# adelacvg/diff-vits

Measured on AMD Instinct MI355X. Metric: mel_frames_per_sec_50step_dpmsolver, higher is better.
Workload: dtype bf16x3 (bf16 MFMA operands split hi+lo, 3 products, fp32 accumulate / fp32 activations); 1 GPU; B=8/GPU, C=80, T=1024, L=256, 50-step DPM-Solver++(2M) multistep, UNet1DConditionModel (128, 256, 384, 512), seeded random-init weights; global_batch=8, concurrent_sub_batches_per_gpu=1, rccl_world_size=1, parallelism=dp1 (batch-sharded, RCCL broadcast of conditioning + all-gather of mels)

## Files before the change

diff-vits_amd/_lib.py:

```python
import ctypes as C
import os
import subprocess

_HERE = os.path.dirname(os.path.abspath(__file__))
LIB_PATH = os.environ.get("DVITS_LIB_FILE") or os.path.join(_HERE, "libdvits_hip.so")
CSRC = os.path.join(_HERE, "csrc")

PREC_BF16X3, PREC_BF16 = 0, 1
SOLVER_DPMPP, SOLVER_UNIPC_BH1, SOLVER_UNIPC_BH2, SOLVER_UNIPC_VARY = 0, 1, 2, 3
SKIP = {"time_uniform": 0, "time_quadratic": 1, "logSNR": 2}
SCHEDULE = {"discrete": 0, "linear": 1, "cosine": 2}
METHOD = {"multistep": 0, "singlestep": 1, "singlestep_fixed": 2}


class UNetCfg(C.Structure):
    _fields_ = [("in_channels", C.c_int32), ("out_channels", C.c_int32), ("n_levels", C.c_int32),
                ("block_out_channels", C.c_int32 * 6), ("layers_per_block", C.c_int32), ("num_heads", C.c_int32),
                ("cross_attention_dim", C.c_int32), ("norm_num_groups", C.c_int32), ("add_embed_heads", C.c_int32),
                ("norm_eps", C.c_float)]


class PencCfg(C.Structure):
    _fields_ = [("in_channels", C.c_int32), ("hidden_channels", C.c_int32), ("out_channels", C.c_int32),
                ("n_layers", C.c_int32), ("num_heads", C.c_int32), ("ffn_kernel", C.c_int32)]
# ... 52 lines not shown
    "dv_sampler_plan_method": (C.c_int, [C.c_int32, C.c_int32, C.c_void_p, C.c_int32, C.c_double, C.c_double, C.c_int32, C.c_int32,
                                         C.c_int32, C.c_int32, C.c_int32, C.c_double, C.c_double, C.c_int32, C.POINTER(C.c_void_p)]),
    "dv_plan_times": (C.c_int, [C.c_void_p, C.POINTER(C.c_int32), C.c_void_p]),
    "dv_plan_destroy": (None, [C.c_void_p]),
    "dv_plan_info": (C.c_int, [C.c_void_p, C.POINTER(C.c_int32), C.c_void_p, C.c_void_p]),
    "dv_plan_coefs": (C.c_int, [C.c_void_p, C.POINTER(C.c_int32), C.c_void_p]),
    "dv_plan_events": (C.c_int, [C.c_void_p, C.POINTER(C.c_int32), C.c_void_p, C.POINTER(C.c_int32)]),
    "dv_sampler_run": (C.c_int, [C.c_void_p, C.c_void_p, C.c_void_p, C.c_void_p, C.c_void_p]),
    "dv_sampler_run_custom": (C.c_int, [C.c_void_p, MODEL_FN, C.c_void_p, C.c_void_p, C.c_int64, C.c_void_p]),
    "dv_plan_set_thresholding": (C.c_int, [C.c_void_p, C.c_double, C.c_double, C.c_void_p]),
    "dv_sampler_run_custom_rows": (C.c_int, [C.c_void_p, MODEL_FN, C.c_void_p, C.c_void_p, C.c_int32, C.c_int64, C.c_void_p]),
    "dv_op_dynamic_threshold": (C.c_int, [C.c_void_p, C.c_int32, C.c_int64, C.c_double, C.c_double, C.c_void_p, C.c_void_p]),
    "dv_plan_set_guidance": (C.c_int, [C.c_void_p, C.c_double, C.c_int32]),
    "dv_op_cfg_combine": (C.c_int, [C.c_void_p, C.c_void_p, C.c_int32, C.c_int64, C.c_double, C.c_void_p]),
    "dv_op_cfg_pair_in": (C.c_int, [C.c_void_p, C.c_void_p, C.c_int64, C.c_void_p]),
    "dv_plan_graph_nodes": (C.c_int, [C.c_void_p, C.POINTER(C.c_int64)]),
    "dv_op_conv1d": (C.c_int, [C.c_void_p, C.c_void_p, C.c_void_p, C.c_void_p] + [C.c_int32] * 8 + [C.c_void_p]),
    "dv_op_linear": (C.c_int, [C.c_void_p, C.c_void_p, C.c_void_p, C.c_void_p] + [C.c_int32] * 4 + [C.c_void_p]),
    "dv_op_linear_planes": (C.c_int, [C.c_void_p] * 6 + [C.c_int32] * 6 + [C.c_void_p]),
    "dv_op_group_stats": (C.c_int, [C.c_void_p, C.c_void_p, C.c_void_p] + [C.c_int32] * 4 + [C.c_float, C.c_void_p]),
    "dv_op_attention": (C.c_int, [C.c_void_p] * 5 + [C.c_int32] * 5 + [C.c_void_p]),
    "dv_op_attention_frag": (C.c_int, [C.c_void_p] * 5 + [C.c_int32] * 5 + [C.c_void_p]),
    "dv_op_conv3": (C.c_int, [C.c_void_p] * 6 + [C.c_int32] * 7 + [C.c_void_p]),
}

_lib = None


def build(force=False, verbose=False):
    if force and os.path.exists(LIB_PATH):
        os.remove(LIB_PATH)
    proc = subprocess.run(["make", "-C", CSRC, "-j", str(min(8, os.cpu_count() or 1))],
                          stdout=subprocess.PIPE, stderr=subprocess.STDOUT, text=True)
    if verbose or proc.returncode != 0:
        print(proc.stdout)
    if proc.returncode != 0 or not os.path.exists(LIB_PATH):
        raise RuntimeError("building libdvits_hip.so failed:\n" + proc.stdout[-4000:])
    return LIB_PATH


def lib():
    global _lib
    if _lib is None:
        if not os.path.exists(LIB_PATH):
            raise RuntimeError("libdvits_hip.so not found at %s — run `python -c 'import __graft_entry__ as g; "
                               "g.build()'` (or `make -C diff-vits_amd/csrc`) first; there is no fallback path"
# ... 31 lines not shown
```

diff-vits_amd/csrc/dv_common.h:

```cpp
#pragma once
#include <hip/hip_runtime.h>
#include <stdint.h>

typedef unsigned short bf16_t;

enum { DV_ZERO_PAGE_BYTES = 32768 };
enum { EPI_STORE = 0, EPI_RESIDUAL = 1, EPI_GEGLU = 2, EPI_STORE_NCT = 3 };
enum { UP_NONE = 0, UP_X2 = 1, UP_SIZE = 2 };

struct GemmSeg {
  const bf16_t* a0_hi; const bf16_t* a0_lo;
  const bf16_t* a1_hi; const bf16_t* a1_lo;
  int c0, c1;
  int taps;
  int pad;
  int nkt;
};

struct GnxParams {
  unsigned long long* xchg;
  unsigned* status;
  const float* gamma; const float* beta;
  const float* tscale; const float* tshift; int ld_t;
  int groups; float eps; int silu;
// ... 185 lines not shown
hipError_t launch_rel_attention(const RelAttnParams& p, hipStream_t st);

enum { POP_GEMM = 0, POP_ATTN = 1, POP_GN = 2, POP_SPLIT = 3 };
struct PersistSync {
  unsigned arrive[8][32];
  unsigned rank[8][32];
  unsigned error;
  unsigned pad_;
  unsigned long long ticks[1024];
};

hipError_t launch_gemm(const GemmParams& p, int precision, hipStream_t st);
hipError_t gemm_init();
bool gemm_conv3_shape_ok(const GemmParams& p);
int gemm_conv3_k(const GemmParams& p);
int gemm_conv3_split(const GemmParams& p, int n_cu);
size_t gemm_conv3_split_bytes(const GemmParams& p);
int gemm_conv3_row_tiles(const GemmParams& p, int bm);
hipError_t conv3_init();
void conv3_env_refresh();
hipError_t launch_conv3(const GemmParams& p, hipStream_t st);
bool gemm_conv3_up_ok(const GemmParams& p);
hipError_t launch_conv3_up(const GemmParams& p, hipStream_t st);
void gemm_env_refresh();
hipError_t attn_init();
hipError_t launch_attention(const AttnParams& p, hipStream_t st);

hipError_t launch_pack_input(const float* x, int cx, const float* cond, int cc, bf16_t* out_hi, bf16_t* out_lo, int cpad,
                             int B, int T, hipStream_t st,
                             unsigned long long* reset = nullptr, size_t reset_words = 0, int Tp = 0);
hipError_t launch_split(const float* in, bf16_t* hi, bf16_t* lo, int64_t n, hipStream_t st);
struct GnApplyParams {
  const float* a0; const float* a1; int c0, c1;
  const float* slab0; const float* slab1;
  const float* st16_0; const float* st16_1;
  const float* scale_in; const float* shift_in;
  const float* gamma; const float* beta; float eps; int groups;
  const float* tscale; const float* tshift; int ld_t;
  int silu;
  bf16_t* out_hi; bf16_t* out_lo; bf16_t* raw_hi; bf16_t* raw_lo;
  int B, T;
  int Tv;
};
hipError_t launch_gn_apply(const GnApplyParams& p, hipStream_t st);

struct PersistOp {
// ... 64 lines not shown
```

diff-vits_amd/csrc/engine.hip:

```cpp
#include "../../include/dvits_hip.h"
#include "dv_common.h"

#include <atomic>
#include <cmath>
#include <cstdarg>
#include <cstdio>
#include <cstdlib>
#include <cstring>
#include <functional>
#include <map>
#include <memory>
#include <string>
#include <type_traits>
#include <vector>

static thread_local char g_err[1024] = "";
int dv_fail(int code, const char* fmt, ...) {
  va_list ap;
  va_start(ap, fmt);
  vsnprintf(g_err, sizeof(g_err), fmt, ap);
  va_end(ap);
  return code;
}
extern "C" const char* dv_last_error(void) { return g_err; }
// ... 596 lines not shown
  }
  bool ff_split_on = [] { const char* e = getenv("DVITS_FF_SPLIT"); return !(e && e[0] == '0'); }();
  bool chain_ff_on = [] { const char* e = getenv("DVITS_CHAIN_FF"); return !(e && e[0] == '0'); }();
  bool chain_split_on = [] { const char* e = getenv("DVITS_CHAIN_SPLIT"); return !(e && e[0] == '0'); }();
  bool chain_xsplit_on = [] { const char* e = getenv("DVITS_CHAIN_XSPLIT"); return !(e && e[0] == '0'); }();
  bool qkv_split_on = [] { const char* e = getenv("DVITS_QKV_SPLIT"); return !(e && e[0] == '0'); }();
  int qkv_split_min_wg = [] { const char* e = getenv("DVITS_QKV_SPLIT_MIN_WG"); return e ? atoi(e) : 96; }();
  int qkv_split_min_c = [] { const char* e = getenv("DVITS_QKV_SPLIT_MIN_C"); return e ? atoi(e) : 256; }();
  bool qkv_xa_on = [] { const char* e = getenv("DVITS_QKV_XA"); return !(e && e[0] == '0'); }();
  int qkv_xa_min_c = [] { const char* e = getenv("DVITS_QKV_XA_MIN_C"); return e ? atoi(e) : 256; }();
  int ff_split_min_wg = [] { const char* e = getenv("DVITS_FF_SPLIT_MIN_WG"); return e ? atoi(e) : 96; }();
  bool gnx_ff_on = [] { const char* e = getenv("DVITS_GNX_FF"); return !(e && e[0] == '0'); }();
  bool cat_drop_fp32 = [] { const char* e = getenv("DVITS_GNX_CONCAT_KEEP_FP32"); return !(e && e[0] == '1'); }();

  int conv3_min_tiles = [] { const char* e = getenv("DVITS_CONV3_MIN_TILES"); return e ? atoi(e) : 64; }();
  int conv3_route(const GemmParams& g) const {
    if (arena.exact || autotune_on() || prec != DV_PREC_BF16X3) return 0;
    GemmParams t = g;
    t.B = B;
    if (gemm_conv3_up_ok(t)) {
      const int tu = gemm_conv3_row_tiles(t, 128) * (t.N / 64);
      return tu >= (conv3_min_tiles < 64 ? conv3_min_tiles : 96) ? 2 : 0;
    }
    if (!gemm_conv3_shape_ok(t)) return 0;
    return gemm_conv3_row_tiles(t, 64) * (t.N / 64) >= conv3_min_tiles ? 1 : 0;
  }
  bool conv3_takes(const GemmParams& g) const { return conv3_route(g) != 0; }
  void gemm(std::vector<OpFn>& ops, GemmParams g, const PackedW* pw, int k_real) {
    g.w_hi = pw->hi; g.w_lo = pw->lo; g.Kp = pw->Kp; g.N_pad = pw->N_pad;
    if (!g.bias) g.bias = pw->bias;
    g.B = B;
    g.zero_page = u->zero_page;
    const int p = prec;
    const int route = conv3_route(g);
    const bool c3 = route != 0 && (dry || g.Kp == gemm_conv3_k(g)) && frag(pw);
    g.c3_route = c3 ? route : 0;
    if (c3) { g.wf_hi = dry ? reinterpret_cast<const bf16_t*>(0x1000) : pw->fhi; g.wf_lo = dry ? reinterpret_cast<const bf16_t*>(0x1000) : pw->flo; }
    cur_kind = "gemm"; cur_flops = 2.0 * (double)g.M * (double)g.N * (double)k_real;
    {
      char buf[128];
      snprintf(buf, sizeof(buf), "M=%d N=%d K=%d taps=%d nseg=%d epi=%d stride=%d up=%d%s%s%s", g.M, g.N, k_real, g.seg[0].taps,
               g.nseg, g.epi, g.stride, g.up_mode, (g.stats || g.stats16) ? " +stats" : "", c3 ? " resident" : "",
               g.gnx.xchg ? " +gnx" : "");
      cur_desc = buf;
    }
    u->flops += dry ? 0.0 : cur_flops;
// ... 1765 lines not shown
    s.src = w_sc; s.C = Csc; s.taps = 1; s.c_pad = Csc; s.k_off = 3 * Cin;
    HIPCHK(launch_pack_weight(s, hi, lo, Kp, st));
  }
  HIPCHK(launch_relayout_frag(hi, fhi, Npad, Kp, st));
  HIPCHK(launch_relayout_frag(lo, flo, Npad, Kp, st));
  g.seg[0].a0_hi = xh; g.seg[0].a0_lo = xl;
  if (Csc > 0) { g.seg[1].a0_hi = sh; g.seg[1].a0_lo = sl; }
  g.w_hi = hi; g.w_lo = lo; g.wf_hi = fhi; g.wf_lo = flo; g.out = y; g.zero_page = zp;
  if (route == 1) {
    int dev = 0, n_cu = 0;
    (void)hipGetDevice(&dev); (void)hipDeviceGetAttribute(&n_cu, hipDeviceAttributeMultiprocessorCount, dev);
    if (gemm_conv3_split(g, n_cu) == 2 && ((g.M + 31) / 32) * ((g.N + 31) / 32) <= 4096) {
      g.sk_split = 2;
      g.sk_buf = sc.get<float>(gemm_conv3_split_bytes(g), st, false);
      g.sk_ticket = sc.get<unsigned>(4096 * sizeof(unsigned), st, true);
      if (!g.sk_buf || !g.sk_ticket) return dv_fail(DV_ERR_HIP, "dv_op_conv3: hipMalloc failed");
    }
  }
  hipError_t e = launch_gemm(g, DV_PREC_BF16X3, st);
  if (e != hipSuccess) return dv_fail(DV_ERR_HIP, "dv_op_conv3: launch failed: %s", hipGetErrorString(e));
  HIPCHK(hipStreamSynchronize(st));
  return DV_OK;
}
```

diff-vits_amd/csrc/kernels_conv.hip:

```cpp
#include "dv_common.h"
#include "dv_device.h"
#include "gnx_device.h"

#include <cstdlib>
#include <type_traits>

typedef __attribute__((ext_vector_type(8))) __bf16 bf16x8;
typedef __attribute__((ext_vector_type(16))) float f32x16;

#ifdef DV_GEMM_TRACE
__device__ unsigned long long g_c3_trace[1024 * 16];
__device__ int g_c3_sel = 0;
#define DV_C3TRACE(i) do { if (threadIdx.x == 0 && blockIdx.x < 1024 && (g_c3_sel == 0 || g_c3_sel == CIN)) g_c3_trace[blockIdx.x * 16 + (i)] = __builtin_amdgcn_s_memtime(); } while (0)
extern "C" int dv_debug_c3_trace_select(int cin) {
  hipError_t e = hipMemcpyToSymbol(HIP_SYMBOL(g_c3_sel), &cin, sizeof(cin));
  void* d = nullptr;
  if (e == hipSuccess) e = hipGetSymbolAddress(&d, HIP_SYMBOL(g_c3_trace));
  return (int)(e != hipSuccess ? e : hipMemset(d, 0, sizeof(g_c3_trace)));
}
extern "C" int dv_debug_c3_trace(unsigned long long* host, int n_wg) {
  return (int)hipMemcpyFromSymbol(host, HIP_SYMBOL(g_c3_trace), (size_t)n_wg * 16 * sizeof(unsigned long long));
}
#else
#define DV_C3TRACE(i) do {} while (0)
// ... 289 lines not shown
    };
    bf16x8 ah[2][2], al[2][2];
    read_a(0, ah[0], al[0]);
#pragma unroll
    for (int u = 0; u < G::U; ++u) {
      const int cur = u & 1;
      if (u + 1 < G::U) read_a(u + 1, ah[cur ^ 1], al[cur ^ 1]);
      const BFrag f = bq[u % G::DEPTH];
      acc[0] = __builtin_amdgcn_mfma_f32_32x32x16_bf16(f.h, al[cur][0], acc[0], 0, 0, 0);
      acc[1] = __builtin_amdgcn_mfma_f32_32x32x16_bf16(f.h, al[cur][1], acc[1], 0, 0, 0);
      acc[0] = __builtin_amdgcn_mfma_f32_32x32x16_bf16(f.l, ah[cur][0], acc[0], 0, 0, 0);
      acc[1] = __builtin_amdgcn_mfma_f32_32x32x16_bf16(f.l, ah[cur][1], acc[1], 0, 0, 0);
      acc[0] = __builtin_amdgcn_mfma_f32_32x32x16_bf16(f.h, ah[cur][0], acc[0], 0, 0, 0);
      acc[1] = __builtin_amdgcn_mfma_f32_32x32x16_bf16(f.h, ah[cur][1], acc[1], 0, 0, 0);
      __builtin_amdgcn_sched_barrier(0);
      if (u + G::DEPTH < G::U) bq[u % G::DEPTH] = load_unit(u + G::DEPTH);
      __builtin_amdgcn_sched_barrier(0);
    }
  };
  if (kq == 0) run(std::integral_constant<int, 0>{});
  else if (kq == 1) run(std::integral_constant<int, 1>{});
  else if (kq == 2) run(std::integral_constant<int, 2>{});
  else run(std::integral_constant<int, 3>{});
  DV_C3TRACE(3);

  conv3_finish(p, smem, s_bias, s_gnx, acc, rpre, tl, tid, lane, wave, CIN);
}

namespace {
constexpr int BMU = 128, RFU = 4;
template <int CIN>
struct ConvGeomU {
  static constexpr int NCH = CIN / 64, KPT = CIN / 16, KS = 3 * KPT, U = KS / 4;
  static constexpr int DEPTH = U < 6 ? U : 6;
  static constexpr int A_PL = NCH * CHP;
  static constexpr int RED = 2 * 4 * RFU * 4 * 64 * 16;
  static constexpr int SMEM = 2 * A_PL > RED ? 2 * A_PL : RED;
  static_assert(CIN % 64 == 0 && KS % 4 == 0 && SMEM + 4096 <= 160 * 1024, "geometry");
};
}

template <int CIN>
__global__ __launch_bounds__(NT) void k_conv3u(const GemmParams p) {
  using G = ConvGeomU<CIN>;
  extern __shared__ __attribute__((aligned(1024))) char smem[];
  __shared__ __attribute__((aligned(16))) float s_bias[BN];
// ... 443 lines not shown
    const int j = 2 * j2;
    read_a(NCH + j + 1, 1, ahb[1], alb[1]);
    mma(bq[2 * POS], ahb[0], alb[0]);
    __builtin_amdgcn_sched_barrier(0);
    if (!(DV_C3_EXP & 2)) bq[2 * POS] = load_ks(3 * KPT + 4 * (JA + min(j + 6, NC2 - 1)));
    __builtin_amdgcn_sched_barrier(0);
    read_a(NCH + j + 2, 1, ahb[0], alb[0]);
    if (j + 1 < NC2) mma(bq[2 * POS + 1], ahb[1], alb[1]);
    __builtin_amdgcn_sched_barrier(0);
    if (!(DV_C3_EXP & 2)) bq[2 * POS + 1] = load_ks(3 * KPT + 4 * (JA + min(j + 7, NC2 - 1)));
    __builtin_amdgcn_sched_barrier(0);
  };
  for (int j2 = 0; j2 < NS2; j2 += 3) {
    pair(j2, std::integral_constant<int, 0>{});
    if (j2 + 1 < NS2) pair(j2 + 1, std::integral_constant<int, 1>{});
    if (j2 + 2 < NS2) pair(j2 + 2, std::integral_constant<int, 2>{});
  }
  DV_C3TRACE(3);
  conv3_finish(p, smem, s_bias, s_gnx, acc, rpre, tl, tid, lane, wave, CIN);
}

static bool g_conv3_on = true;
static int g_conv3_stream = 512;
void conv3_env_refresh() {
  const char* e = getenv("DVITS_CONV3"); g_conv3_on = !(e && e[0] == '0');
  const char* e2 = getenv("DVITS_CONV3_STREAM"); g_conv3_stream = e2 ? atoi(e2) : 512;
}
static const bool g_conv3_env_once = [] { conv3_env_refresh(); return true; }();

bool gemm_conv3_shape_ok(const GemmParams& p) {
  if (!g_conv3_on || p.nseg < 1 || p.nseg > 2 || p.seg[0].taps != 3 || p.seg[0].pad != 1 || p.stride != 1 || p.up_mode != UP_NONE) return false;
  const int cin = p.seg[0].c0 + p.seg[0].c1;
  if (cin < 128 || cin > 1024 || cin % 128 != 0) return false;
  if (p.seg[0].c0 % 64 != 0 || p.seg[0].c1 % 64 != 0 || (p.seg[0].c1 > 0 && !p.seg[0].a1_hi)) return false;
  if (p.nseg == 2) {
    const GemmSeg& s1 = p.seg[1];
    if (s1.taps != 1 || s1.pad != 0 || s1.c0 <= 0 || s1.c0 % 64 != 0 || s1.c1 % 64 != 0 || (s1.c1 > 0 && !s1.a1_hi) || s1.c0 + s1.c1 > 2048) return false;
  }
  const int tv_out = p.Tv_out > 0 ? p.Tv_out : p.T_out, tv_in = p.Tv_in > 0 ? p.Tv_in : p.T_in;
  if (p.T_in != p.T_out || tv_in != tv_out || p.T_virt != tv_out || tv_out > p.T_out || tv_out <= p.T_out - 32) return false;
  if (p.T_out % 32 != 0 || p.N % BN != 0 || p.B <= 0 || p.M != p.B * p.T_out) return false;
  if ((p.epi != EPI_STORE && p.epi != EPI_RESIDUAL) || p.stats || p.rowstat_out || p.ln_stat || p.relu || p.rowmask) return false;
  if ((p.ldo & 7) != 0 || (p.epi == EPI_RESIDUAL && (p.ldres & 3) != 0) || p.force_tile != GT_AUTO) return false;
  return true;
}
int gemm_conv3_row_tiles(const GemmParams& p, int bm) { return p.B * ((p.T_out + bm - 1) / bm); }
int gemm_conv3_split(const GemmParams& p, int n_cu) {
  static const bool on = [] { const char* e = getenv("DVITS_CONV3_SPLIT"); return !(e && e[0] == '0'); }();
  if (!on || n_cu <= 0 || !gemm_conv3_shape_ok(p)) return 0;
  const int cin = p.seg[0].c0 + p.seg[0].c1, nch = cin >> 6, nc2 = p.nseg > 1 ? (p.seg[1].c0 + p.seg[1].c1) >> 6 : 0;
  if (cin <= 512 && cin <= g_conv3_stream && p.nseg == 1) return 0;
  if (2 * gemm_conv3_row_tiles(p, BM) * (p.N / BN) > n_cu || nch < 4 || nch + ((nc2 + 1) >> 1) < 8) return 0;
  return 2;
}
size_t gemm_conv3_split_bytes(const GemmParams& p) { return (size_t)2 * gemm_conv3_row_tiles(p, BM) * (p.N / BN) * BM * BN * sizeof(float); }
bool gemm_conv3_up_ok(const GemmParams& p) {
  if (!g_conv3_on || p.nseg != 1 || p.seg[0].taps != 3 || p.seg[0].pad != 1 || p.stride != 1 || p.up_mode != UP_X2) return false;
  const int cin = p.seg[0].c0 + p.seg[0].c1;
  if (cin != 128 && cin != 256 && cin != 384 && cin != 512) return false;
  if (p.seg[0].c0 % 64 != 0 || p.seg[0].c1 % 64 != 0 || (p.seg[0].c1 > 0 && !p.seg[0].a1_hi)) return false;
  const int tv_out = p.Tv_out > 0 ? p.Tv_out : p.T_out, tv_in = p.Tv_in > 0 ? p.Tv_in : p.T_in;
  if (tv_out != 2 * tv_in || p.T_virt != tv_out || tv_out > p.T_out || tv_out <= p.T_out - 32 || tv_in > p.T_in) return false;
  if (p.T_out % 32 != 0 || p.N % BN != 0 || p.B <= 0 || p.M != p.B * p.T_out) return false;
  if ((p.epi != EPI_STORE && p.epi != EPI_RESIDUAL) || p.stats || p.rowstat_out || p.ln_stat || p.relu || p.rowmask) return false;
  if ((p.ldo & 7) != 0 || (p.epi == EPI_RESIDUAL && (p.ldres & 3) != 0) || p.force_tile != GT_AUTO || p.sk_buf) return false;
  return true;
}
int gemm_conv3_k(const GemmParams& p) {
  return 3 * (p.seg[0].c0 + p.seg[0].c1) + (p.nseg > 1 ? p.seg[1].c0 + p.seg[1].c1 : 0);
}
static void conv3_geometry(GemmParams& p, int bm) {
  p.c3_tu = (p.T_out + bm - 1) / bm;
  p.c3_tu_magic = p.c3_tu <= 1 ? 0u : (unsigned)(((1ull << 32) + (unsigned)p.c3_tu - 1) / (unsigned)p.c3_tu);
}

template <int CIN>
static hipError_t conv3_launch(const GemmParams& p, hipStream_t st) {
  constexpr int smem = ConvGeom<CIN>::SMEM;
  hipLaunchKernelGGL((k_conv3<CIN>), dim3(gemm_conv3_row_tiles(p, BM) * (p.N / BN)), dim3(NT), smem, st, p);
  return hipGetLastError();
}
template <int CIN>
static hipError_t conv3_attr() {
  return hipFuncSetAttribute(reinterpret_cast<const void*>(k_conv3<CIN>), hipFuncAttributeMaxDynamicSharedMemorySize, ConvGeom<CIN>::SMEM);
}
template <int CIN>
static hipError_t conv3u_attr() {
  return hipFuncSetAttribute(reinterpret_cast<const void*>(k_conv3u<CIN>), hipFuncAttributeMaxDynamicSharedMemorySize, ConvGeomU<CIN>::SMEM);
}
template <int CIN>
static hipError_t conv3u_launch(const GemmParams& p, hipStream_t st) {
  constexpr int smem = ConvGeomU<CIN>::SMEM;
  hipLaunchKernelGGL((k_conv3u<CIN>), dim3(gemm_conv3_row_tiles(p, BMU) * (p.N / BN)), dim3(NT), smem, st, p);
  return hipGetLastError();
}
hipError_t launch_conv3_up(const GemmParams& pin, hipStream_t st) {
  GemmParams p = pin;
  if (!p.wf_hi || !p.wf_lo || !gemm_conv3_up_ok(p) || p.Kp != 3 * (p.seg[0].c0 + p.seg[0].c1) || p.sk_mode != 0) return hipErrorInvalidValue;
  if (p.Tv_out <= 0) p.Tv_out = p.T_out;
  if (p.Tv_in <= 0) p.Tv_in = p.T_in;
  conv3_geometry(p, BMU);
  if (p.xcd_n > 0) p.xcd_n = 0;
  switch (p.seg[0].c0 + p.seg[0].c1) {
    case 128: return conv3u_launch<128>(p, st);
    case 256: return conv3u_launch<256>(p, st);
    case 384: return conv3u_launch<384>(p, st);
    default: return conv3u_launch<512>(p, st);
  }
}
hipError_t conv3_init() {
  hipError_t e;
  if ((e = conv3u_attr<128>()) != hipSuccess) return e;
  if ((e = conv3u_attr<256>()) != hipSuccess) return e;
  if ((e = conv3u_attr<384>()) != hipSuccess) return e;
  if ((e = conv3u_attr<512>()) != hipSuccess) return e;
  if ((e = hipFuncSetAttribute(reinterpret_cast<const void*>(k_conv3s), hipFuncAttributeMaxDynamicSharedMemorySize, S_TOTAL)) != hipSuccess) return e;
  if ((e = conv3_attr<128>()) != hipSuccess) return e;
  if ((e = conv3_attr<256>()) != hipSuccess) return e;
  if ((e = conv3_attr<384>()) != hipSuccess) return e;
  return conv3_attr<512>();
}
hipError_t launch_conv3(const GemmParams& pin, hipStream_t st) {
  GemmParams p = pin;
  if (!p.wf_hi || !p.wf_lo || !gemm_conv3_shape_ok(p) || p.Kp != gemm_conv3_k(p) || (p.sk_mode != 0 && p.sk_mode != 3)) return hipErrorInvalidValue;
  if (p.Tv_out <= 0) p.Tv_out = p.T_out;
  if (p.Tv_in <= 0) p.Tv_in = p.T_in;
  conv3_geometry(p, BM);
  const int tiles = gemm_conv3_row_tiles(p, BM) * (p.N / BN);
  if (p.sk_mode == 3) {
    if (!p.sk_buf || !p.sk_ticket || p.sk_split != 2 || p.seg[0].c0 + p.seg[0].c1 < 256) return hipErrorInvalidValue;
    hipLaunchKernelGGL(k_conv3s, dim3(2 * tiles), dim3(NT_S), S_TOTAL, st, p);
    return hipGetLastError();
  }
  const int cin = p.seg[0].c0 + p.seg[0].c1;
  if (cin > 512 || cin > g_conv3_stream || p.nseg > 1) {
    hipLaunchKernelGGL(k_conv3s, dim3(tiles), dim3(NT_S), S_TOTAL, st, p);
    return hipGetLastError();
  }
  switch (cin) {
// ... 7 lines not shown
```

diff-vits_amd/csrc/kernels_gemm.hip:

```cpp
#include "dv_common.h"
#define DV_GEMM_TRACE_OWNER
#include "gemm_tile.h"

#include <cstdio>
#include <cstdlib>
#include <type_traits>

template <int BM, int BN, int BK, int WM, int WN, int NSPLIT, int KS>
__global__ __launch_bounds__(64 * WM * WN * KS) void k_gemm(const GemmParams p) {
  extern __shared__ __attribute__((aligned(1024))) char smem[];
  asm volatile("" ::"s"(p.seg[0].a0_hi), "s"(p.seg[1].a0_hi), "s"(p.seg[1].pad), "s"(p.T_in), "s"(p.w_hi), "s"(p.M), "s"(p.res),
               "s"(p.out_hi), "s"(p.zero_page), "s"(p.ln_u), "s"(p.gnx.xchg), "s"(p.gnx.y_hi), "s"(p.xcd_n), "s"(p.xcd_inv_tn));
  const int n_tiles_n = (p.N + BN - 1) / BN;
  const int nwg = gridDim.x;
  int bid = blockIdx.x;
  int tm0, tn0, ksel = 0;
  if (p.xcd_n > 0) {
    const int x = bid & 7, i = bid >> 3;
    const int ks_i = x >> p.xcd_sh_mn, r = x & ((1 << p.xcd_sh_mn) - 1), xm_i = r >> p.xcd_sh_n, xn_i = r & (p.xcd_n - 1);
    const int lm = (i * p.xcd_inv_tn) >> 16, ln = i - lm * p.xcd_tn;
    tm0 = (xm_i * p.xcd_tm + lm) * BM; tn0 = (xn_i * p.xcd_tn + ln) * BN; ksel = ks_i;
  } else {
    {
      const int q = nwg >> 3, r = nwg & 7, xcd = bid & 7;
// ... 183 lines not shown
    auto lg2 = [](int v) { int s2 = 0; while ((1 << s2) < v) ++s2; return s2; };
    p.xcd_n = best_xn; p.xcd_sh_n = lg2(best_xn); p.xcd_sh_mn = lg2(xm * best_xn);
    p.xcd_tn = tn / best_xn; p.xcd_tm = tm / xm; p.xcd_inv_tn = (65536 + p.xcd_tn - 1) / p.xcd_tn;
  }
}
static int gemm_utt_tiles_per_xcd(const GemmParams& p, int tu, int tm, int tn) {
  if (p.xcd_n > 0) return (tu < p.xcd_tm ? tu : p.xcd_tm) * p.xcd_tn;
  const int q = (tm * tn + 7) / 8;
  return tu * tn < q ? tu * tn : q;
}

bool gemm_handover_rounds() {
  static const bool on = [] { const char* e = getenv("DVITS_GNX_ROUNDS"); return !(e && e[0] == '0'); }();
  return on;
}
int gemm_gnx_plan(const GemmParams& p, int n_cu) {
  if (p.force_tile != GT_AUTO || (p.epi != EPI_STORE && p.epi != EPI_RESIDUAL) || !p.stats16 || p.rowmask || p.relu) return 0;
  const int skc = p.gnx.sk_c;
  if (p.M != p.B * p.T_out || p.gnx.groups <= 0 || p.gnx.groups > 64 || skc < 0 || (p.N + skc) % p.gnx.groups != 0) return 0;
  const int cpg = (p.N + skc) / p.gnx.groups;
  if (cpg % 16 != 0 || p.N % 16 != 0 || skc % 16 != 0) return 0;
  int bm, bn, tu;
  if (p.c3_route) {
    bm = p.c3_route == 2 ? 128 : 64; bn = 64;
    if (p.T_out % 32 != 0 || p.N % bn != 0) return 0;
    tu = (p.T_out + bm - 1) / bm;
  } else {
    gemm_pick_tile(p, bm, bn);
    if (p.T_out % bm != 0 || p.N % bn != 0) return 0;
    tu = p.T_out / bm;
  }
  if (skc > 0 && ((skc / 16 + p.N / bn - 1) / (p.N / bn)) * 16 > 128) return 0;
  if ((p.T_out / 32) * (cpg / 16) > 256) return 0;
  const int tm = p.B * tu, tn = p.N / bn, tiles = tm * tn;
  const bool pair = p.sk_buf && p.sk_split == 2 && p.sk_ticket;
  if (p.sk_buf && !pair) return 0;
  if (pair) {
    if (2 * tiles > n_cu) return 0;
  } else if (tiles > n_cu) {
    if (!gemm_handover_rounds() || n_cu < 8) return 0;
    GemmParams t = p;
    if (p.c3_route == 2) t.xcd_n = 0; else gemm_xcd_rect(t, tm, tn, 1);
    if (gemm_utt_tiles_per_xcd(t, tu, tm, tn) > n_cu / 8) return 0;
  }
  return (p.M / 32) * (p.N / 16);
}

// ... 14 lines not shown
      for (int s2 = 0; s2 < p.nseg; ++s2) k += p.seg[s2].taps * (p.seg[s2].c0 + p.seg[s2].c1);
      snprintf(g_trace_desc, sizeof(g_trace_desc), "M=%d N=%d K=%d taps=%d nseg=%d epi=%d stride=%d up=%d%s%s%s%s%s%s split=%d%s",
               p.M, p.N, k, p.seg[0].taps, p.nseg, p.epi, p.stride, p.up_mode, p.stats ? " +colstats" : "", p.stats16 ? " +stats16" : "",
               p.gnx.xchg ? " +gnx" : "", p.out_hi ? " +planes" : "", p.rowstat_out ? " +rowstat" : "", p.ln_stat ? " +ln" : "",
               p.sk_buf ? p.sk_split : 0, (p.sk_buf && p.sk_ticket && p.sk_split == 2) ? "f" : "");
    }
    ++g_trace_no;
  }
#endif
  const bool x3 = precision == 0;
  if (!p.zero_page || (x3 && !p.w_lo)) return hipErrorInvalidValue;
  if (p.Tv_out <= 0) p.Tv_out = p.T_out;
  if (p.Tv_in <= 0) p.Tv_in = p.T_in;
  if (p.Tv_out > p.T_out || p.Tv_in > p.T_in || ((p.stats16 || p.gnx.xchg) && p.Tv_out <= p.T_out - 32)) return hipErrorInvalidValue;
  if (p.T_out < 1 || (unsigned long long)(p.M > 0 ? p.M : 1) * (unsigned long long)p.T_out >= (1ull << 32)) return hipErrorInvalidValue;
  p.tout_magic = gemm_tout_magic(p.T_out);
  if (p.ln_stat && (p.ln_nblk < 1 || p.ln_nblk > 16)) return hipErrorInvalidValue;
  for (int s2 = 0; s2 < p.nseg; ++s2)
    if (2 * (size_t)p.seg[s2].c0 + 256 > DV_ZERO_PAGE_BYTES || 2 * (size_t)p.seg[s2].c1 + 256 > DV_ZERO_PAGE_BYTES) return hipErrorInvalidValue;
  p.c3_route = 0;
  if (x3 && p.wf_hi && p.wf_lo) {
    if (gemm_conv3_shape_ok(p) && p.Kp == gemm_conv3_k(p)) p.c3_route = 1;
    else if (gemm_conv3_up_ok(p) && p.Kp == 3 * (p.seg[0].c0 + p.seg[0].c1)) p.c3_route = 2;
  }
  if (p.gnx.xchg && p.sk_mode == 0) {
    static const int n_cu = [] { int d = 0, n = 0; (void)hipGetDevice(&d); (void)hipDeviceGetAttribute(&n, hipDeviceAttributeMultiprocessorCount, d); return n; }();
    if (!p.gnx.status || !p.gnx.y_hi || !p.gnx.gamma || !p.gnx.beta || gemm_gnx_plan(p, n_cu) <= 0) return hipErrorInvalidValue;
    if (p.gnx.sk_c > 0 && (!p.gnx.sk_x || !p.gnx.sk_stat16 || !p.gnx.sk_y_hi || (x3 && !p.gnx.sk_y_lo) || p.gnx.tscale)) return hipErrorInvalidValue;
  }
  if (p.sk_buf && p.sk_split == 2 && p.sk_ticket && p.sk_mode == 0) {
    p.sk_mode = 3;
    return launch_gemm(p, precision, st);
  }
  if (p.sk_buf && p.sk_split >= 2 && p.sk_mode == 0) {
    p.sk_mode = 1;
    hipError_t e = launch_gemm(p, precision, st);
    if (e != hipSuccess) return e;
    p.sk_mode = 2;
    return launch_gemm(p, precision, st);
  }
  if (!p.sk_buf || p.sk_split < 2) { p.sk_buf = nullptr; p.sk_split = 0; p.sk_mode = 0; p.sk_ticket = nullptr; }
  const bool c3 = p.c3_route == 1 && (p.sk_mode == 0 || p.sk_mode == 3);
  p.xcd_n = 0;
  if (p.force_tile == GT_AUTO) {
    int bm, bn;
    gemm_pick_tile(p, bm, bn);
    const int tm = c3 ? gemm_conv3_row_tiles(p, 64) : (p.M + bm - 1) / bm, tn = c3 ? p.N / 64 : (p.N + bn - 1) / bn;
    const int xs = (p.sk_mode == 1 || p.sk_mode == 3) ? p.sk_split : 1;
    gemm_xcd_rect(p, tm, tn, xs);
  }
  if (c3) return launch_conv3(p, st);
  if (p.c3_route == 2 && p.sk_mode == 0) return launch_conv3_up(p, st);
  const GemmTune& tune = gemm_tune();
  const int big_tiles = ((p.M + 127) / 128) * ((p.N + 127) / 128);
  bool k64 = tune.bk64 != 0;
  for (int s = 0; s < p.nseg; ++s) k64 = k64 && p.seg[s].c0 % 64 == 0 && p.seg[s].c1 % 64 == 0;
  const int ft = p.force_tile & 0xff;
  if (ft != GT_AUTO && (p.force_tile & GT_BK64) && !k64) return hipErrorInvalidValue;
  const bool big = ft != GT_AUTO ? ft == GT_T0 : big_tiles >= tune.big;
  const int bk = ft != GT_AUTO ? ((p.force_tile & GT_BK64) ? 64 : 32) : ((!big && k64) ? 64 : 32);
  for (int s = 0; s < p.nseg; ++s) {
    if (p.seg[s].c0 % 32 != 0 || p.seg[s].c1 % 32 != 0) return hipErrorInvalidValue;
    p.seg[s].nkt = p.seg[s].taps * (p.seg[s].c0 + p.seg[s].c1) / bk;
  }
  if (ft != GT_AUTO) return bk == 64 ? Tiles<64>::launch_forced(p, x3, ft, st) : Tiles<32>::launch_forced(p, x3, ft, st);
  if (big) return tune.ksplit ? Tiles<32>::T0::launch(p, x3, st) : Tiles<32>::T0S::launch(p, x3, st);
  if (bk == 64) return Tiles<64>::launch(p, x3, tune.min_wg, tune.ksplit != 0, st);
  return Tiles<32>::launch(p, x3, tune.min_wg > 0 ? tune.min_wg : 1, false, st);
}
```

include/dvits_hip.h:

```cpp
#ifndef DVITS_HIP_H
#define DVITS_HIP_H

#include <stdint.h>

#ifdef __cplusplus
extern "C" {
#endif

typedef enum {
  DV_OK = 0,
  DV_ERR_INVALID = -1,
  DV_ERR_HIP = -2,
  DV_ERR_STATE = -3,
  DV_ERR_MISSING_WEIGHT = -4
} dv_status;

typedef enum { DV_PREC_BF16X3 = 0, DV_PREC_BF16 = 1 } dv_precision;

typedef struct {
  int32_t in_channels;
  int32_t out_channels;
  int32_t n_levels;
  int32_t block_out_channels[6];
  int32_t layers_per_block;
// ... 116 lines not shown
int dv_tenc_forward(dv_tenc* t, const int64_t* ids, const int64_t* tone, const int64_t* language, const int64_t* lengths,
                    const float* g, float* x, float* m, float* logs, void* stream);
int dv_tenc_stats(dv_tenc* t, int64_t* n_launch, double* flops);
int dv_tenc_probe(dv_tenc* t, const char* name, float* host_out, int64_t capacity, int64_t* dims);


int dv_op_rel_attention(const float* q, const float* k, const float* v, const float* emb_k, const float* emb_v,
                        const int64_t* lengths, float* o, int32_t B, int32_t H, int32_t T, int32_t d, int32_t window, void* stream);

int dv_op_conv1d(const float* x, const float* w, const float* bias, float* y, int32_t B, int32_t Cin, int32_t T,
                 int32_t Cout, int32_t k, int32_t stride, int32_t up_T, int32_t precision, void* stream);
int dv_op_linear(const float* x, const float* w, const float* bias, float* y, int32_t M, int32_t K, int32_t N,
                 int32_t precision, void* stream);
int dv_op_linear_planes(const float* x, const float* w, const float* bias, float* y, uint16_t* y_hi, uint16_t* y_lo, int32_t M,
                        int32_t K, int32_t N, int32_t ldo, int32_t geglu, int32_t precision, void* stream);
int dv_op_group_stats(const float* x, float* mean, float* rstd, int32_t B, int32_t T, int32_t C, int32_t groups,
                      float eps, void* stream);
int dv_op_attention(const float* q, const float* k, const float* v, const float* bias, float* o, int32_t B,
                    int32_t H, int32_t Tq, int32_t Tk, int32_t d, void* stream);
int dv_op_attention_frag(const float* q, const float* k, const float* v, const float* bias, float* o, int32_t B,
                         int32_t H, int32_t Tq, int32_t Tk, int32_t d, void* stream);
int dv_op_conv3(const float* x, const float* w, const float* bias, const float* x_sc, const float* w_sc, float* y, int32_t B,
                int32_t Cin, int32_t T, int32_t Tp, int32_t Cout, int32_t Csc, int32_t up2, void* stream);
int dv_op_dynamic_threshold(float* x0_inout, int32_t rows, int64_t row_numel, double ratio, double max_val, float* s_out,
                            void* stream);
int dv_op_cfg_combine(const float* x0_pair, float* out, int32_t rows, int64_t row_numel, double scale, void* stream);
int dv_op_cfg_pair_in(const float* in, float* out, int64_t numel, void* stream);

#ifdef __cplusplus
}
#endif
#endif
```

Measured before the change: 68120 mel-frames/s.

## Add dedicated stride-2 conv3 kernel for UNet downsample convolutions

Adds k_conv3d, a resident-weight MFMA kernel specialised for stride-2, kernel-3 downsampling convolutions (Cin 128/256/384). It stages even and odd input rows in LDS so all three taps reuse them, and streams pre-relayouted bf16x3 weight fragments through a register queue. Previously these convs fell through to the generic k_gemm path. The engine routes them to the new kernel (c3_route=3) when enough tiles exist, and a standalone test entry point is added. It brings more template instances and tile-count thresholds that may leave some shapes underfilling the GPU.

```diff
diff --git a/diff-vits_amd/_lib.py b/diff-vits_amd/_lib.py
--- a/diff-vits_amd/_lib.py
+++ b/diff-vits_amd/_lib.py
@@ -98,6 +98,7 @@
     "dv_op_attention": (C.c_int, [C.c_void_p] * 5 + [C.c_int32] * 5 + [C.c_void_p]),
     "dv_op_attention_frag": (C.c_int, [C.c_void_p] * 5 + [C.c_int32] * 5 + [C.c_void_p]),
     "dv_op_conv3": (C.c_int, [C.c_void_p] * 6 + [C.c_int32] * 7 + [C.c_void_p]),
+    "dv_op_conv3_down": (C.c_int, [C.c_void_p] * 9 + [C.c_int32] * 7 + [C.c_void_p]),
 }
 
 _lib = None
diff --git a/diff-vits_amd/csrc/dv_common.h b/diff-vits_amd/csrc/dv_common.h
--- a/diff-vits_amd/csrc/dv_common.h
+++ b/diff-vits_amd/csrc/dv_common.h
@@ -231,6 +231,9 @@
 hipError_t launch_conv3(const GemmParams& p, hipStream_t st);
 bool gemm_conv3_up_ok(const GemmParams& p);
 hipError_t launch_conv3_up(const GemmParams& p, hipStream_t st);
+bool gemm_conv3_down_ok(const GemmParams& p);
+int gemm_conv3_down_bm(const GemmParams& p);
+hipError_t launch_conv3_down(const GemmParams& p, hipStream_t st);
 void gemm_env_refresh();
 hipError_t attn_init();
 hipError_t launch_attention(const AttnParams& p, hipStream_t st);
diff --git a/diff-vits_amd/csrc/engine.hip b/diff-vits_amd/csrc/engine.hip
--- a/diff-vits_amd/csrc/engine.hip
+++ b/diff-vits_amd/csrc/engine.hip
@@ -642,6 +642,8 @@
       const int tu = gemm_conv3_row_tiles(t, 128) * (t.N / 64);
       return tu >= (conv3_min_tiles < 64 ? conv3_min_tiles : 96) ? 2 : 0;
     }
+    if (gemm_conv3_down_ok(t))
+      return gemm_conv3_row_tiles(t, gemm_conv3_down_bm(t)) * (t.N / 64) >= conv3_min_tiles ? 3 : 0;
     if (!gemm_conv3_shape_ok(t)) return 0;
     return gemm_conv3_row_tiles(t, 64) * (t.N / 64) >= conv3_min_tiles ? 1 : 0;
   }
@@ -2453,3 +2455,66 @@
   HIPCHK(hipStreamSynchronize(st));
   return DV_OK;
 }
+
+extern "C" int dv_op_conv3_down(const float* x, const float* w, const float* bias, float* y, float* stat16, const float* gamma,
+                                const float* beta, uint16_t* yn_hi, uint16_t* yn_lo, int32_t B, int32_t C, int32_t T, int32_t Tp,
+                                int32_t Cout, int32_t groups, int32_t resident, void* stream) {
+  if (!x || !w || !y || B <= 0 || C <= 0 || T <= 0 || Tp < T || Cout <= 0 || C % 64 != 0 || Cout % 16 != 0)
+    return dv_fail(DV_ERR_INVALID, "dv_op_conv3_down: bad argument");
+  if (gamma && (!beta || !stat16 || !yn_hi || !yn_lo || groups <= 0)) return dv_fail(DV_ERR_INVALID, "dv_op_conv3_down: the in-launch GroupNorm needs beta, stat16, both planes and groups");
+  if (2 * (size_t)C + 256 > DV_ZERO_PAGE_BYTES) return dv_fail(DV_ERR_INVALID, "dv_op_conv3_down: C = %d exceeds one source tensor's width", C);
+  hipStream_t st = (hipStream_t)stream;
+  HIPCHK(gemm_init());
+  gemm_env_refresh();
+  HIPCHK(attn_init());
+  const int Kp = 3 * C, Npad = rup(Cout, 128), Tv_out = (T + 1) / 2, T_out = rup(Tv_out, 32);
+  GemmParams g{};
+  g.nseg = 1; g.B = B;
+  g.T_in = Tp; g.Tv_in = g.T_virt = T; g.T_out = T_out; g.Tv_out = Tv_out;
+  g.stride = 2; g.up_mode = UP_NONE;
+  g.M = B * T_out; g.N = Cout; g.epi = EPI_STORE; g.ldo = Cout; g.ldres = Cout; g.Kp = Kp; g.N_pad = Npad; g.bias = bias;
+  g.seg[0].c0 = C; g.seg[0].taps = 3; g.seg[0].pad = 1;
+  g.stats16 = stat16;
+  if (resident && !gemm_conv3_down_ok(g))
+    return dv_fail(DV_ERR_INVALID, "dv_op_conv3_down: B=%d C=%d T=%d Tp=%d Cout=%d is not a shape of the stride-2 convolution kernel "
+                   "(it would run on k_gemm)", B, C, T, Tp, Cout);
+  OpScratch sc;
+  const size_t xe = (size_t)B * Tp * C, we = (size_t)Npad * Kp;
+  bf16_t* xh = sc.get<bf16_t>(xe * 2, st, false); bf16_t* xl = sc.get<bf16_t>(xe * 2, st, false);
+  bf16_t* hi = sc.get<bf16_t>(we * 2, st, true); bf16_t* lo = sc.get<bf16_t>(we * 2, st, true);
+  bf16_t* fhi = sc.get<bf16_t>(we * 2, st, false); bf16_t* flo = sc.get<bf16_t>(we * 2, st, false);
+  bf16_t* zp = sc.get<bf16_t>(DV_ZERO_PAGE_BYTES, st, true);
+  if (!xh || !xl || !hi || !lo || !fhi || !flo || !zp) return dv_fail(DV_ERR_HIP, "dv_op_conv3_down: hipMalloc failed");
+  HIPCHK(launch_split(x, xh, xl, (int64_t)xe, st));
+  PackSpec s{};
+  s.src = w; s.N = Cout; s.kind = 1; s.C = C; s.taps = 3; s.c_pad = C; s.k_off = 0; s.n_off = 0;
+  HIPCHK(launch_pack_weight(s, hi, lo, Kp, st));
+  HIPCHK(launch_relayout_frag(hi, fhi, Npad, Kp, st));
+  HIPCHK(launch_relayout_frag(lo, flo, Npad, Kp, st));
+  g.seg[0].a0_hi = xh; g.seg[0].a0_lo = xl;
+  g.w_hi = hi; g.w_lo = lo; g.out = y; g.zero_page = zp;
+  if (resident) { g.wf_hi = fhi; g.wf_lo = flo; g.c3_route = 3; }
+  unsigned* status = nullptr;
+  if (gamma) {
+    int dev = 0, n_cu = 0;
+    (void)hipGetDevice(&dev); (void)hipDeviceGetAttribute(&n_cu, hipDeviceAttributeMultiprocessorCount, dev);
+    g.gnx.groups = groups;
+    const int nw = gemm_gnx_plan(g, n_cu);
+    if (nw <= 0) return dv_fail(DV_ERR_INVALID, "dv_op_conv3_down: the in-launch GroupNorm cannot be planned for this shape");
+    g.gnx.xchg = sc.get<unsigned long long>((size_t)nw * 8, st, false);
+    status = sc.get<unsigned>(64, st, true);
+    if (!g.gnx.xchg || !status) return dv_fail(DV_ERR_HIP, "dv_op_conv3_down: hipMalloc failed");
+    HIPCHK(hipMemsetAsync(g.gnx.xchg, 0xff, (size_t)nw * 8, st));
+    g.gnx.status = status; g.gnx.gamma = gamma; g.gnx.beta = beta; g.gnx.eps = 1e-5f; g.gnx.silu = 0; g.gnx.spin_max = 1 << 18;
+    g.gnx.y_hi = yn_hi; g.gnx.y_lo = yn_lo;
+  }
+  hipError_t e = launch_gemm(g, DV_PREC_BF16X3, st);
+  if (e != hipSuccess) return dv_fail(DV_ERR_HIP, "dv_op_conv3_down: launch failed: %s", hipGetErrorString(e));
+  HIPCHK(hipStreamSynchronize(st));
+  if (status) {
+    unsigned flag = 0;
+    HIPCHK(hipMemcpy(&flag, status, sizeof(flag), hipMemcpyDeviceToHost));
+    if (flag) return dv_fail(DV_ERR_HIP, "dv_op_conv3_down: the in-launch GroupNorm hand-over timed out");
+  }
+  return DV_OK;
+}
diff --git a/diff-vits_amd/csrc/kernels_conv.hip b/diff-vits_amd/csrc/kernels_conv.hip
--- a/diff-vits_amd/csrc/kernels_conv.hip
+++ b/diff-vits_amd/csrc/kernels_conv.hip
@@ -335,6 +335,153 @@
   else if (kq == 1) run(std::integral_constant<int, 1>{});
   else if (kq == 2) run(std::integral_constant<int, 2>{});
   else run(std::integral_constant<int, 3>{});
+  DV_C3TRACE(3);
+
+  conv3_finish(p, smem, s_bias, s_gnx, acc, rpre, tl, tid, lane, wave, CIN);
+}
+
+namespace {
+template <int CIN, int BMD>
+struct ConvGeomD {
+  static constexpr int NCH = CIN / 64, KPT = CIN / 16, KS = 3 * KPT, U = KS / 4;
+  static constexpr int RF = BMD / 32;
+  static constexpr int DEPTH = U < 8 ? U : 8;
+  static constexpr int NG = BMD / 4 + 1;
+  static constexpr int ROWS_D = 8 * NG;
+  static constexpr int CHP_D = ROWS_D * 128;
+  static constexpr int A_PL = NCH * CHP_D;
+  static constexpr int SMEM = 2 * A_PL > RED_BYTES ? 2 * A_PL : RED_BYTES;
+  static_assert(CIN % 64 == 0 && KS % 4 == 0 && (BMD == 32 || BMD == 64) && SMEM + 4096 <= 160 * 1024, "geometry");
+};
+}
+
+template <int CIN, int BMD>
+__global__ __launch_bounds__(NT) void k_conv3d(const GemmParams p) {
+  using G = ConvGeomD<CIN, BMD>;
+  extern __shared__ __attribute__((aligned(1024))) char smem[];
+  __shared__ __attribute__((aligned(16))) float s_bias[BN];
+  __shared__ GnxShared<BN> s_gnx;
+  asm volatile("" ::"s"(p.seg[0].a0_hi), "s"(p.seg[1].a0_hi), "s"(p.seg[1].pad), "s"(p.T_in), "s"(p.w_hi), "s"(p.M), "s"(p.res),
+               "s"(p.out_hi), "s"(p.zero_page), "s"(p.ln_u), "s"(p.gnx.xchg), "s"(p.gnx.y_hi), "s"(p.xcd_n), "s"(p.xcd_inv_tn), "s"(p.wf_lo));
+  DV_C3TRACE(0);
+  C3Tile tl;
+  conv3_tile(p, tl, BMD);
+  const int m0 = tl.m0, n0 = tl.n0, t0 = tl.t0;
+  const int tid = threadIdx.x, lane = tid & 63, wave = __builtin_amdgcn_readfirstlane(tid >> 6);
+  const int l31 = lane & 31, lh = lane >> 5;
+  const int cf = wave & 1, kq = wave >> 1;
+  const int e_wn = cf, e_wm = (wave >> 1) & 1, e_half = wave >> 2;
+  const unsigned a_base = (unsigned)(size_t)smem;
+  const GemmSeg& sg = p.seg[0];
+  const int c0 = sg.c0;
+  const int m_last = p.M - 1;
+
+  float rpre[8];
+  if (p.epi == EPI_RESIDUAL) {
+    const float* rp = p.res + (size_t)min(m0 + e_wm * 32 + l31, m_last) * p.ldres + n0 + e_wn * 32 + e_half * 16 + 4 * lh;
+#pragma unroll
+    for (int g = 0; g < 2; ++g) {
+      const float4 a = *reinterpret_cast<const float4*>(rp + 8 * g);
+      rpre[4 * g] = a.x; rpre[4 * g + 1] = a.y; rpre[4 * g + 2] = a.z; rpre[4 * g + 3] = a.w;
+    }
+  }
+  if (wave == 0) glds4(p.bias ? (const void*)(p.bias + n0 + lane) : (const void*)p.zero_page, (unsigned)(size_t)s_bias);
+  {
+    const int lr = lane >> 3, slot = lane & 7;
+    const size_t ms0 = (size_t)tl.bq * p.T_in;
+#pragma unroll
+    for (int gi = 0; gi < (G::NG + NWV - 1) / NWV; ++gi) {
+      const int g = wave + gi * NWV;
+      if (g < G::NG) {
+        const int r = g * 8 + lr;
+        const int f = r < BMD ? 2 * t0 + 2 * r : 2 * t0 + 2 * (r - BMD) - 1;
+        const bool ok = r <= 2 * BMD && f >= 0 && f < p.Tv_in;
+        const int sc8 = (slot ^ swz(r)) << 3;
+        const size_t e = ok ? (ms0 + (size_t)f) * c0 + sc8 : 0;
+#pragma unroll
+        for (int c = 0; c < G::NCH; ++c) {
+          const unsigned dst = a_base + (unsigned)(c * G::CHP_D + g * 1024);
+          glds16(ok ? (const void*)(sg.a0_hi + e + c * 64) : (const void*)p.zero_page, dst);
+          glds16(ok ? (const void*)(sg.a0_lo + e + c * 64) : (const void*)p.zero_page, dst + G::A_PL);
+        }
+      }
+    }
+  }
+  const size_t w_e0 = ((size_t)((n0 >> 5) + cf) * G::KS + (size_t)kq * G::U) * 512 + (size_t)lane * 8;
+  const bf16_t* const wh = p.wf_hi + w_e0;
+  const bf16_t* const wl = p.wf_lo + w_e0;
+  auto load_unit = [&](int j) {
+    BFrag f;
+    f.h = *reinterpret_cast<const bf16x8*>(wh + (size_t)j * 512);
+    f.l = *reinterpret_cast<const bf16x8*>(wl + (size_t)j * 512);
+    return f;
+  };
+  BFrag bq[G::DEPTH];
+#pragma unroll
+  for (int j = 0; j < G::DEPTH; ++j) bq[j] = load_unit(j);
+  __builtin_amdgcn_sched_barrier(0);
+  DV_C3TRACE(1);
+  wait_vmcnt<2 * G::DEPTH>();
+  __syncthreads();
+  DV_C3TRACE(2);
+
+  int rowb[G::RF][3], swl[G::RF][3];
+#pragma unroll
+  for (int rf = 0; rf < G::RF; ++rf)
+#pragma unroll
+    for (int tap = 0; tap < 3; ++tap) {
+      const int j = rf * 32 + l31, row = tap == 1 ? j : BMD + j + (tap >> 1);
+      rowb[rf][tap] = row * 128;
+      swl[rf][tap] = swz(row) ^ lh;
+    }
+  f32x16 acc[2];
+#pragma unroll
+  for (int rf = 0; rf < 2; ++rf)
+#pragma unroll
+    for (int r = 0; r < 16; ++r) acc[rf][r] = 0.f;
+  auto run = [&](auto kq_tag) __attribute__((always_inline)) {
+    constexpr int KQ = decltype(kq_tag)::value;
+    auto read_a = [&](int u, bf16x8 (&h)[G::RF], bf16x8 (&l)[G::RF]) {
+      const int ks = KQ * G::U + u, tap = ks / G::KPT, cs = ks - tap * G::KPT;
+#pragma unroll
+      for (int rf = 0; rf < G::RF; ++rf) {
+        const int off = (cs >> 2) * G::CHP_D + rowb[rf][tap] + ((((cs & 3) << 1) ^ swl[rf][tap]) << 4);
+        h[rf] = *reinterpret_cast<const bf16x8*>(smem + off);
+        l[rf] = *reinterpret_cast<const bf16x8*>(smem + G::A_PL + off);
+      }
+    };
+    bf16x8 ah[2][G::RF], al[2][G::RF];
+    read_a(0, ah[0], al[0]);
+#pragma unroll
+    for (int u = 0; u < G::U; ++u) {
+      const int cur = u & 1;
+      if (u + 1 < G::U) read_a(u + 1, ah[cur ^ 1], al[cur ^ 1]);
+      const BFrag f = bq[u % G::DEPTH];
+      if constexpr (G::RF == 2) {
+        acc[0] = __builtin_amdgcn_mfma_f32_32x32x16_bf16(f.h, al[cur][0], acc[0], 0, 0, 0);
+        acc[1] = __builtin_amdgcn_mfma_f32_32x32x16_bf16(f.h, al[cur][1], acc[1], 0, 0, 0);
+        acc[0] = __builtin_amdgcn_mfma_f32_32x32x16_bf16(f.l, ah[cur][0], acc[0], 0, 0, 0);
+        acc[1] = __builtin_amdgcn_mfma_f32_32x32x16_bf16(f.l, ah[cur][1], acc[1], 0, 0, 0);
+        acc[0] = __builtin_amdgcn_mfma_f32_32x32x16_bf16(f.h, ah[cur][0], acc[0], 0, 0, 0);
+        acc[1] = __builtin_amdgcn_mfma_f32_32x32x16_bf16(f.h, ah[cur][1], acc[1], 0, 0, 0);
+      } else {
+        acc[1] = __builtin_amdgcn_mfma_f32_32x32x16_bf16(f.h, al[cur][0], acc[1], 0, 0, 0);
+        acc[0] = __builtin_amdgcn_mfma_f32_32x32x16_bf16(f.h, ah[cur][0], acc[0], 0, 0, 0);
+        acc[1] = __builtin_amdgcn_mfma_f32_32x32x16_bf16(f.l, ah[cur][0], acc[1], 0, 0, 0);
+      }
+      __builtin_amdgcn_sched_barrier(0);
+      if (u + G::DEPTH < G::U) bq[u % G::DEPTH] = load_unit(u + G::DEPTH);
+      __builtin_amdgcn_sched_barrier(0);
+    }
+  };
+  if (kq == 0) run(std::integral_constant<int, 0>{});
+  else if (kq == 1) run(std::integral_constant<int, 1>{});
+  else if (kq == 2) run(std::integral_constant<int, 2>{});
+  else run(std::integral_constant<int, 3>{});
+  if constexpr (G::RF == 1) {
+#pragma unroll
+    for (int r = 0; r < 16; ++r) { acc[0][r] += acc[1][r]; acc[1][r] = 0.f; }
+  }
   DV_C3TRACE(3);
 
   conv3_finish(p, smem, s_bias, s_gnx, acc, rpre, tl, tid, lane, wave, CIN);
@@ -824,8 +971,10 @@
 
 static bool g_conv3_on = true;
 static int g_conv3_stream = 512;
+static bool g_conv3_down = true;
 void conv3_env_refresh() {
   const char* e = getenv("DVITS_CONV3"); g_conv3_on = !(e && e[0] == '0');
+  const char* e3 = getenv("DVITS_CONV3_DOWN"); g_conv3_down = !(e3 && e3[0] == '0');
   const char* e2 = getenv("DVITS_CONV3_STREAM"); g_conv3_stream = e2 ? atoi(e2) : 512;
 }
 static const bool g_conv3_env_once = [] { conv3_env_refresh(); return true; }();
@@ -868,6 +1017,18 @@
   if ((p.ldo & 7) != 0 || (p.epi == EPI_RESIDUAL && (p.ldres & 3) != 0) || p.force_tile != GT_AUTO || p.sk_buf) return false;
   return true;
 }
+bool gemm_conv3_down_ok(const GemmParams& p) {
+  if (!g_conv3_on || !g_conv3_down || p.nseg != 1 || p.seg[0].taps != 3 || p.seg[0].pad != 1 || p.stride != 2 || p.up_mode != UP_NONE) return false;
+  const int cin = p.seg[0].c0;
+  if ((cin != 128 && cin != 256 && cin != 384) || p.seg[0].c1 != 0) return false;
+  const int tv_out = p.Tv_out > 0 ? p.Tv_out : p.T_out, tv_in = p.Tv_in > 0 ? p.Tv_in : p.T_in;
+  if (tv_in < 1 || tv_in > p.T_in || p.T_virt != tv_in || tv_out != (tv_in + 1) / 2 || tv_out > p.T_out || tv_out <= p.T_out - 32) return false;
+  if (p.T_out % 32 != 0 || p.N % BN != 0 || p.B <= 0 || p.M != p.B * p.T_out) return false;
+  if ((p.epi != EPI_STORE && p.epi != EPI_RESIDUAL) || p.stats || p.rowstat_out || p.ln_stat || p.relu || p.rowmask) return false;
+  if ((p.ldo & 7) != 0 || (p.epi == EPI_RESIDUAL && (p.ldres & 3) != 0) || p.force_tile != GT_AUTO || p.sk_buf) return false;
+  return true;
+}
+int gemm_conv3_down_bm(const GemmParams& p) { return p.seg[0].c0 <= 256 ? 64 : 32; }
 int gemm_conv3_k(const GemmParams& p) {
   return 3 * (p.seg[0].c0 + p.seg[0].c1) + (p.nseg > 1 ? p.seg[1].c0 + p.seg[1].c1 : 0);
 }
@@ -895,6 +1056,28 @@
   constexpr int smem = ConvGeomU<CIN>::SMEM;
   hipLaunchKernelGGL((k_conv3u<CIN>), dim3(gemm_conv3_row_tiles(p, BMU) * (p.N / BN)), dim3(NT), smem, st, p);
   return hipGetLastError();
+}
+template <int CIN, int BMD>
+static hipError_t conv3d_attr() {
+  return hipFuncSetAttribute(reinterpret_cast<const void*>(k_conv3d<CIN, BMD>), hipFuncAttributeMaxDynamicSharedMemorySize, ConvGeomD<CIN, BMD>::SMEM);
+}
+template <int CIN, int BMD>
+static hipError_t conv3d_launch(const GemmParams& p, hipStream_t st) {
+  constexpr int smem = ConvGeomD<CIN, BMD>::SMEM;
+  hipLaunchKernelGGL((k_conv3d<CIN, BMD>), dim3(gemm_conv3_row_tiles(p, BMD) * (p.N / BN)), dim3(NT), smem, st, p);
+  return hipGetLastError();
+}
+hipError_t launch_conv3_down(const GemmParams& pin, hipStream_t st) {
+  GemmParams p = pin;
+  if (!p.wf_hi || !p.wf_lo || !gemm_conv3_down_ok(p) || p.Kp != 3 * p.seg[0].c0 || p.sk_mode != 0) return hipErrorInvalidValue;
+  if (p.Tv_out <= 0) p.Tv_out = p.T_out;
+  if (p.Tv_in <= 0) p.Tv_in = p.T_in;
+  conv3_geometry(p, gemm_conv3_down_bm(p));
+  switch (p.seg[0].c0) {
+    case 128: return conv3d_launch<128, 64>(p, st);
+    case 256: return conv3d_launch<256, 64>(p, st);
+    default: return conv3d_launch<384, 32>(p, st);
+  }
 }
 hipError_t launch_conv3_up(const GemmParams& pin, hipStream_t st) {
   GemmParams p = pin;
@@ -917,6 +1100,9 @@
   if ((e = conv3u_attr<384>()) != hipSuccess) return e;
   if ((e = conv3u_attr<512>()) != hipSuccess) return e;
   if ((e = hipFuncSetAttribute(reinterpret_cast<const void*>(k_conv3s), hipFuncAttributeMaxDynamicSharedMemorySize, S_TOTAL)) != hipSuccess) return e;
+  if ((e = conv3d_attr<128, 64>()) != hipSuccess) return e;
+  if ((e = conv3d_attr<256, 64>()) != hipSuccess) return e;
+  if ((e = conv3d_attr<384, 32>()) != hipSuccess) return e;
   if ((e = conv3_attr<128>()) != hipSuccess) return e;
   if ((e = conv3_attr<256>()) != hipSuccess) return e;
   if ((e = conv3_attr<384>()) != hipSuccess) return e;
diff --git a/diff-vits_amd/csrc/kernels_gemm.hip b/diff-vits_amd/csrc/kernels_gemm.hip
--- a/diff-vits_amd/csrc/kernels_gemm.hip
+++ b/diff-vits_amd/csrc/kernels_gemm.hip
@@ -229,7 +229,7 @@
   if (cpg % 16 != 0 || p.N % 16 != 0 || skc % 16 != 0) return 0;
   int bm, bn, tu;
   if (p.c3_route) {
-    bm = p.c3_route == 2 ? 128 : 64; bn = 64;
+    bm = p.c3_route == 2 ? 128 : (p.c3_route == 3 ? gemm_conv3_down_bm(p) : 64); bn = 64;
     if (p.T_out % 32 != 0 || p.N % bn != 0) return 0;
     tu = (p.T_out + bm - 1) / bm;
   } else {
@@ -290,6 +290,7 @@
   if (x3 && p.wf_hi && p.wf_lo) {
     if (gemm_conv3_shape_ok(p) && p.Kp == gemm_conv3_k(p)) p.c3_route = 1;
     else if (gemm_conv3_up_ok(p) && p.Kp == 3 * (p.seg[0].c0 + p.seg[0].c1)) p.c3_route = 2;
+    else if (gemm_conv3_down_ok(p) && p.Kp == 3 * p.seg[0].c0) p.c3_route = 3;
   }
   if (p.gnx.xchg && p.sk_mode == 0) {
     static const int n_cu = [] { int d = 0, n = 0; (void)hipGetDevice(&d); (void)hipDeviceGetAttribute(&n, hipDeviceAttributeMultiprocessorCount, d); return n; }();
@@ -309,16 +310,19 @@
   }
   if (!p.sk_buf || p.sk_split < 2) { p.sk_buf = nullptr; p.sk_split = 0; p.sk_mode = 0; p.sk_ticket = nullptr; }
   const bool c3 = p.c3_route == 1 && (p.sk_mode == 0 || p.sk_mode == 3);
+  const bool c3d = p.c3_route == 3 && p.sk_mode == 0;
   p.xcd_n = 0;
   if (p.force_tile == GT_AUTO) {
     int bm, bn;
     gemm_pick_tile(p, bm, bn);
-    const int tm = c3 ? gemm_conv3_row_tiles(p, 64) : (p.M + bm - 1) / bm, tn = c3 ? p.N / 64 : (p.N + bn - 1) / bn;
+    const int tm = c3 ? gemm_conv3_row_tiles(p, 64) : c3d ? gemm_conv3_row_tiles(p, gemm_conv3_down_bm(p)) : (p.M + bm - 1) / bm;
+    const int tn = (c3 || c3d) ? p.N / 64 : (p.N + bn - 1) / bn;
     const int xs = (p.sk_mode == 1 || p.sk_mode == 3) ? p.sk_split : 1;
     gemm_xcd_rect(p, tm, tn, xs);
   }
   if (c3) return launch_conv3(p, st);
   if (p.c3_route == 2 && p.sk_mode == 0) return launch_conv3_up(p, st);
+  if (c3d) return launch_conv3_down(p, st);
   const GemmTune& tune = gemm_tune();
   const int big_tiles = ((p.M + 127) / 128) * ((p.N + 127) / 128);
   bool k64 = tune.bk64 != 0;
diff --git a/include/dvits_hip.h b/include/dvits_hip.h
--- a/include/dvits_hip.h
+++ b/include/dvits_hip.h
@@ -162,6 +162,9 @@
                          int32_t H, int32_t Tq, int32_t Tk, int32_t d, void* stream);
 int dv_op_conv3(const float* x, const float* w, const float* bias, const float* x_sc, const float* w_sc, float* y, int32_t B,
                 int32_t Cin, int32_t T, int32_t Tp, int32_t Cout, int32_t Csc, int32_t up2, void* stream);
+int dv_op_conv3_down(const float* x, const float* w, const float* bias, float* y, float* stat16, const float* gamma, const float* beta,
+                     uint16_t* yn_hi, uint16_t* yn_lo, int32_t B, int32_t C, int32_t T, int32_t Tp, int32_t Cout, int32_t groups,
+                     int32_t resident, void* stream);
 int dv_op_dynamic_threshold(float* x0_inout, int32_t rows, int64_t row_numel, double ratio, double max_val, float* s_out,
                             void* stream);
 int dv_op_cfg_combine(const float* x0_pair, float* out, int32_t rows, int64_t row_numel, double scale, void* stream);
```

Result: no change. 68100 mel-frames/s (-0.0%).
